# PeterFWS/Structure-PLP-SLAM

Measured on AMD Instinct MI355X. Metric: frames/sec ORB+LSD extract+match, 640x480 TUM-RGBD, 1/2/4/8 GPU, higher is better.
Workload: dtype u8

## Files before the change

structure-plp-slam_amd/csrc/match_kernels.hip:

```cpp
#include <hip/hip_runtime.h>
#include <stdint.h>
#include <cstdlib>

#include "libstdcxx_sort.hpp"
#include "plp_barrier.hpp"
#include "match_device.hpp"
#include "plp_common.hpp"
#include "xcd_map.hpp"

namespace plp {

__device__ __forceinline__ int floor_d(double v) { int i = (int)v; return i - (i > v); }
__device__ __forceinline__ int ceil_d(double v) { int i = (int)v; return i + (i < v); }

__device__ __forceinline__ unsigned hamming256(const uint4& a0, const uint4& a1, const uint4& b0, const uint4& b1) {
    return __popc(a0.x ^ b0.x) + __popc(a0.y ^ b0.y) + __popc(a0.z ^ b0.z) + __popc(a0.w ^ b0.w) +
           __popc(a1.x ^ b1.x) + __popc(a1.y ^ b1.y) + __popc(a1.z ^ b1.z) + __popc(a1.w ^ b1.w);
}

__device__ __forceinline__ unsigned long long wave_min_u64(unsigned long long v) {
#pragma unroll
    for (int o = 32; o > 0; o >>= 1) {
        const unsigned lo = __shfl_xor((unsigned)v, o), hi = __shfl_xor((unsigned)(v >> 32), o);
        const unsigned long long w = ((unsigned long long)hi << 32) | lo;
        v = w < v ? w : v;
    }
    return v;
}

struct QueryCtx {
    float rx, ry, mg, xr, xr2;
    int min_level, max_level, min_cx, max_cx, min_cy, max_cy;
    double l0, l1, l2, lden;
    double rdx, rdy;
    int group;
    unsigned pred;
    double g0, g1, g2, gden;
    double b1x, b1y, b1z, thr;
    bool stereo;
    bool windowed, empty, line;
};
__device__ __forceinline__ bool is_line_mode(int mode) { return mode == PLP_MATCH_MODE_LANDMARKS_LINE || mode == PLP_MATCH_MODE_LAST_FRAME_LINE || mode == PLP_MATCH_MODE_FUSE_LINE; }
__device__ __forceinline__ bool is_group_mode(int mode) { return mode == PLP_MATCH_MODE_BOW || mode == PLP_MATCH_MODE_TRIANGULATION; }
__device__ __forceinline__ bool is_last_frame_mode(int mode) { return mode == PLP_MATCH_MODE_LAST_FRAME || mode == PLP_MATCH_MODE_LAST_FRAME_LINE; }

template <int FAM>
__device__ __forceinline__ int fam_mode(int m) {
    if constexpr (FAM == kFamLine) return m == PLP_MATCH_MODE_LANDMARKS_LINE ? PLP_MATCH_MODE_LANDMARKS_LINE : PLP_MATCH_MODE_LAST_FRAME_LINE;
    else if constexpr (FAM == kFamGroup) return m == PLP_MATCH_MODE_BOW ? PLP_MATCH_MODE_BOW : PLP_MATCH_MODE_TRIANGULATION;
    else if constexpr (FAM == kFamPoint) return m == PLP_MATCH_MODE_LANDMARKS ? PLP_MATCH_MODE_LANDMARKS : m == PLP_MATCH_MODE_LAST_FRAME ? PLP_MATCH_MODE_LAST_FRAME : PLP_MATCH_MODE_BRUTE_FORCE;
    else if constexpr (FAM == kFamGrid) return m == PLP_MATCH_MODE_LANDMARKS ? PLP_MATCH_MODE_LANDMARKS : PLP_MATCH_MODE_LAST_FRAME;
    else return m;
}

__device__ __forceinline__ int query_direction(const MatchProblem& P, int b) {
    typedef const __attribute__((address_space(1))) int32_t* g_i32;
    return P.directions ? ((g_i32)P.directions)[b] : P.direction;
}

template <int FAM = kFamAny>
__device__ __forceinline__ QueryCtx make_query(const MatchProblem& P, int q, int b, int dir) {
    const int mode = fam_mode<FAM>(P.mode);
    const size_t qoff = (size_t)b * P.m_cap;
    const float* reproj = P.q_reproj ? P.q_reproj + qoff * 2 : nullptr;
    const float* q_xr = P.q_x_right ? P.q_x_right + qoff : nullptr;
    const int32_t* q_level = P.q_level ? P.q_level + qoff : nullptr;
    QueryCtx c{};
    c.windowed = mode != PLP_MATCH_MODE_BRUTE_FORCE && !is_group_mode(mode);
    c.line = is_line_mode(mode);
    if (is_group_mode(mode)) c.group = P.q_group[qoff + q];
    if (mode == PLP_MATCH_MODE_TRIANGULATION) {
        const double* bq = P.q_bearing + (qoff + q) * 3;
        c.b1x = bq[0]; c.b1y = bq[1]; c.b1z = bq[2];
        c.stereo = q_xr && 0 <= q_xr[q];
        c.thr = (0.2 * 3.14159265358979323846 / 180.0) * (double)P.scale_factors[q_level[q] & 15];
    }
    if (!c.windowed) return c;
    const int lvl = q_level[q];
    const int lvl_tab = min(max(lvl, 0), max(P.num_levels, 1) - 1);
    if (c.line) {
        c.mg = __fmul_rn(P.margin, P.scale_factors[lvl_tab]);
        double x1, y1, x2, y2;
        if (mode == PLP_MATCH_MODE_FUSE_LINE) {
            const double* a = P.q_reproj_d + (qoff + q) * 2; const double* e = P.q_reproj2_d + (qoff + q) * 2;
            x1 = (float)a[0]; y1 = (float)a[1]; x2 = (float)e[0]; y2 = (float)e[1];
            c.g0 = a[1] * 1.0 - 1.0 * e[1]; c.g1 = 1.0 * e[0] - a[0] * 1.0; c.g2 = a[0] * e[1] - a[1] * e[0];
            c.gden = sqrt(c.g0 * c.g0 + c.g1 * c.g1);
        } else {
            const float* r2 = P.q_reproj2 + qoff * 2;
            x1 = reproj[2 * q]; y1 = reproj[2 * q + 1]; x2 = r2[2 * q]; y2 = r2[2 * q + 1];
        }
        c.l0 = y1 * 1.0 - 1.0 * y2; c.l1 = 1.0 * x2 - x1 * 1.0; c.l2 = x1 * y2 - y1 * x2;
        c.lden = sqrt(c.l0 * c.l0 + c.l1 * c.l1);
        c.xr = q_xr ? q_xr[q] : -1.f;
        c.xr2 = P.q_x_right2 ? P.q_x_right2[qoff + q] : -1.f;
        if (mode == PLP_MATCH_MODE_FUSE_LINE) { c.min_level = -1; c.max_level = -1; }
        else if (mode == PLP_MATCH_MODE_LANDMARKS_LINE || P.level_window == 1) { c.min_level = lvl - 1; c.max_level = lvl; }
        else if (P.level_window == 2) { c.min_level = lvl - 1; c.max_level = lvl + 1; }
        else {
            if (dir == 1) { c.min_level = lvl; c.max_level = P.num_levels_lsd; }
            else if (dir == 2) { c.min_level = 0; c.max_level = lvl + 1; }
            else { c.min_level = lvl - 1; c.max_level = lvl + 1; }
        }
        c.empty = false;
        return c;
    }
    if (mode == PLP_MATCH_MODE_FUSE) {
        const double* rd = P.q_reproj_d + qoff * 2;
        c.rdx = rd[2 * q]; c.rdy = rd[2 * q + 1];
        c.rx = (float)c.rdx; c.ry = (float)c.rdy;
        c.pred = (unsigned)lvl;
    } else { c.rx = reproj[2 * q]; c.ry = reproj[2 * q + 1]; }
    c.mg = __fmul_rn(P.margin, P.scale_factors[lvl_tab]);
    c.xr = q_xr ? q_xr[q] : -1.f;
    if (mode == PLP_MATCH_MODE_LANDMARKS || (mode == PLP_MATCH_MODE_LAST_FRAME && P.level_window == 1)) { c.min_level = lvl - 1; c.max_level = lvl; }
    else if (mode == PLP_MATCH_MODE_FUSE) { c.min_level = -1; c.max_level = -1; }
    else if (P.level_window == 2) { c.min_level = lvl - 1; c.max_level = lvl + 1; }
    else {
        if (dir == 1) { c.min_level = lvl; c.max_level = P.num_levels - 1; }
        else if (dir == 2) { c.min_level = 0; c.max_level = lvl; }
        else { c.min_level = lvl - 1; c.max_level = lvl + 1; }
    }
    c.min_cx = max(0, floor_d((double)__fsub_rn(__fsub_rn(c.rx, P.grid_min_x), c.mg) * P.inv_cell_w));
    c.max_cx = min(P.grid_cols - 1, ceil_d((double)__fadd_rn(__fsub_rn(c.rx, P.grid_min_x), c.mg) * P.inv_cell_w));
    c.min_cy = max(0, floor_d((double)__fsub_rn(__fsub_rn(c.ry, P.grid_min_y), c.mg) * P.inv_cell_h));
    c.max_cy = min(P.grid_rows - 1, ceil_d((double)__fadd_rn(__fsub_rn(c.ry, P.grid_min_y), c.mg) * P.inv_cell_h));
    c.empty = P.grid_cols <= c.min_cx || c.max_cx < 0 || P.grid_rows <= c.min_cy || c.max_cy < 0;
    if (mode == PLP_MATCH_MODE_LAST_FRAME && (P.flags & PLP_MATCH_FLAG_UNSIGNED_LEVEL) && lvl == 0) c.empty = true;
    return c;
}

struct LineTarget { float sx, sy, ex, ey; int octave; bool occ; float xr, xr2; unsigned kp_oct; };
template <int FAM = kFamAny>
__device__ __forceinline__ bool line_gate(const MatchProblem& P, const QueryCtx& c, const LineTarget& T, bool has_xr) {
    const int mode = fam_mode<FAM>(P.mode);
    const float dsp = (float)(((double)T.sx * c.l0 + (double)T.sy * c.l1 + c.l2) / c.lden);
    const float dep = (float)(((double)T.ex * c.l0 + (double)T.ey * c.l1 + c.l2) / c.lden);
    if (fabsf(dsp) > c.mg || fabsf(dep) > c.mg) return false;
    const bool check_level = (0 < c.min_level) || (0 <= c.max_level);
    if (check_level) {
        if (T.octave < c.min_level) return false;
        if (c.max_level > 0 && T.octave > c.max_level) return false;
    }
    if (T.occ) return false;
    if (mode == PLP_MATCH_MODE_LAST_FRAME_LINE && P.is_rgbd && has_xr && P.t_x_right2) {
        const float a = T.xr, b2 = T.xr2;
        if (a > 0 && b2 > 0 && (c.mg < fabsf(__fsub_rn(c.xr, a)) || c.mg < fabsf(__fsub_rn(c.xr2, b2)))) return false;
    }
    return true;
}

template <int FAM = kFamAny>
__device__ __forceinline__ unsigned long long candidate_key(const MatchProblem& P, const QueryCtx& c, int t, const plp_keypoint* kps,
                                                           const uint8_t* t_desc, const float* t_xr, const uint8_t* t_occ,
                                                           const uint4& q0, const uint4& q1) {
    const int mode = fam_mode<FAM>(P.mode);
    unsigned order = (unsigned)t, oct = 0;
    if (is_group_mode(mode)) {
        const size_t tb = (size_t)(t_desc - P.t_desc) / 32;
// ... 403 lines not shown
#pragma unroll
                for (int e = kMatchK - 1; e > 0; --e) { const uint32_t lo = min(ovf[e], ovf[e - 1]), hi = max(ovf[e], ovf[e - 1]); ovf[e - 1] = lo; ovf[e] = hi; }
            }
        };
        int passed = 0;
        float rx = 0.f, ry = 0.f, mg = 0.f, qxr = 0.f;
        uint32_t win = 1u, lvls = 255u << 16;
        int i = 0, i1 = 0;
        uint4 q0 = make_uint4(0u, 0u, 0u, 0u), q1 = q0;
        if (active) {
            const QueryCtx c = make_query(P, q, b, s_dir);
            if (!c.empty) {
                const uint4* qd = reinterpret_cast<const uint4*>(P.q_desc + ((size_t)b * P.q_desc_stride + q) * 32);
                q0 = qd[0]; q1 = qd[1];
                rx = c.rx; ry = c.ry; mg = c.mg; qxr = c.xr;
                win = (uint32_t)c.min_cx | ((uint32_t)c.max_cx << 8) | ((uint32_t)c.min_cy << 16) | ((uint32_t)c.max_cy << 24);
                lvls = (uint32_t)min(max(c.min_level, 0), 256) | ((c.max_level < 0 ? 255u : (uint32_t)min(c.max_level, 255)) << 16);
            }
        }
        bool wave_more;
        do {
            uint32_t pend[kLanePend / 2];
#pragma unroll
            for (int k = 0; k < kLanePend / 2; ++k) pend[k] = 0u;
            int nc = 0;
            for (;;) {
                if (i >= i1) {
                    const int col = (int)(win & 0xffu);
                    if (col <= (int)((win >> 8) & 0xffu)) {
                        i = cs[col * rows + (int)((win >> 16) & 0xffu)]; i1 = cs[col * rows + (int)(win >> 24) + 1];
                        ++win;
                    }
                } else {
                    const int p = i++;
                    const float2 sp = t_xy(p);
                    const uint32_t oct = t_to(p) >> 16;
                    bool ok = (lvls & 0xffffu) <= oct && oct <= (lvls >> 16) && fabsf(__fsub_rn(sp.x, rx)) < mg && fabsf(__fsub_rn(sp.y, ry)) < mg;
                    if (ok && has_xr) {
                        const float xr = t_xr(p);
                        ok = !(0 < xr && mg < fabsf(__fsub_rn(qxr, xr)));
                    }
                    if (ok) {
                        const uint32_t v = (uint32_t)p << (16 * (nc & 1));
#pragma unroll
                        for (int k = 0; k < kLanePend / 2; ++k) pend[k] |= (nc >> 1) == k ? v : 0u;
                        ++nc;
                    }
                }
                wave_more = __builtin_amdgcn_ballot_w64(i < i1 || (win & 0xffu) <= ((win >> 8) & 0xffu)) != 0ull;
                if (!wave_more || __builtin_amdgcn_ballot_w64(nc == kLanePend) != 0ull) break;
            }
            auto slot_pos = [&](int j) -> int { return (int)((pend[j >> 1] >> (16 * (j & 1))) & 0xffffu); };
            auto gather = [&](int j, uint4& a0, uint4& a1) {
                if (j < nc) {
                    const uint4* d = reinterpret_cast<const uint4*>(t_desc + 32 * (size_t)(t_to(slot_pos(j)) & 0xffffu));
                    a0 = d[0]; a1 = d[1];
                }
            };
            uint4 a0 = make_uint4(0u, 0u, 0u, 0u), a1 = a0;
            gather(0, a0, a1);
#pragma unroll
            for (int j = 0; j < kLanePend; ++j) {
                if (__builtin_amdgcn_ballot_w64(j < nc) == 0ull) break;
                uint4 b0 = a0, b1 = a1;
                if (j + 1 < kLanePend) gather(j + 1, b0, b1);
                if (j < nc) insert((hamming256(q0, q1, a0, a1) << 16) | (uint32_t)slot_pos(j));
                a0 = b0; a1 = b1;
            }
            passed += nc;
        } while (wave_more);
        if (!in_range) continue;
        uint32_t e[kMatchK];
#pragma unroll
        for (int k = 0; k < kMatchK; ++k) {
            e[k] = 0xffffffffu;
            if (top[k] != 0xffffffffu) {
                const uint32_t to = t_to((int)(top[k] & 0xffffu));
                e[k] = ((top[k] >> 16) << 20) | (((to >> 16) & 15u) << 16) | (to & 0xffffu);
            }
        }
        static_assert(kMatchK == 8, "two 16-byte stores per query");
        uint4* out = reinterpret_cast<uint4*>(P.klist + ((size_t)b * P.m_cap + q) * kMatchK);
        out[0] = make_uint4(e[0], e[1], e[2], e[3]);
        out[1] = make_uint4(e[4], e[5], e[6], e[7]);
        P.kcount[(size_t)b * P.m_cap + q] = active ? passed : -1;
        if (passed > kMatchK) {
#pragma unroll
            for (int k = 0; k < kMatchK; ++k) {
                e[k] = 0xffffffffu;
                if (ovf[k] != 0xffffffffu) {
                    const uint32_t to = t_to((int)(ovf[k] & 0xffffu));
                    e[k] = ((ovf[k] >> 16) << 20) | (((to >> 16) & 15u) << 16) | (to & 0xffffu);
                }
            }
            uint4* out2 = reinterpret_cast<uint4*>(P.klist2 + ((size_t)b * P.m_cap + q) * kMatchK);
            out2[0] = make_uint4(e[0], e[1], e[2], e[3]);
            out2[1] = make_uint4(e[4], e[5], e[6], e[7]);
        }
    }
}

__global__ __launch_bounds__(256) void k_match_topk_lds(MatchProblem P) {
    extern __shared__ __attribute__((aligned(16))) uint8_t smem[];
    const int tid = threadIdx.x, lane = tid & 63, wv = __builtin_amdgcn_readfirstlane(tid >> 6), b = blockIdx.y;
    const int m = P.q_counts ? min(P.q_counts[b], P.m_cap) : P.m_cap;
    const int q_begin = blockIdx.x * kQueriesPerBlock;
    if (q_begin >= m) return;
    const int n = P.t_counts ? min(P.t_counts[b], P.n_cap) : P.n_cap;
    const uint8_t* t_desc = P.t_desc + (size_t)b * P.n_cap * 32;
    uint4* sdesc = reinterpret_cast<uint4*>(smem);
    {
        const uint4* src = reinterpret_cast<const uint4*>(t_desc);
        for (int i = tid; i < 2 * n; i += 256) sdesc[i] = src[i];
    }
    wg_barrier();
    const uint8_t* q_valid = P.q_valid ? P.q_valid + (size_t)b * P.m_cap : nullptr;
    for (int q = q_begin + wv; q < min(m, q_begin + kQueriesPerBlock); q += 4) {
        uint32_t* klist = P.klist + ((size_t)b * P.m_cap + q) * kMatchK;
        int32_t* kcount = P.kcount + (size_t)b * P.m_cap + q;
        if (q_valid && !q_valid[q]) { if (lane == 0) *kcount = -1; continue; }
        const uint4* qd = reinterpret_cast<const uint4*>(P.q_desc + ((size_t)b * P.q_desc_stride + q) * 32);
        const uint4 q0 = qd[0], q1 = qd[1];
        unsigned long long top[kMatchK];
#pragma unroll
        for (int i = 0; i < kMatchK; ++i) top[i] = ~0ull;
        int passed = 0;
        for (int t = lane; t < n; t += 64) {
            const unsigned dist = hamming256(q0, q1, sdesc[2 * t], sdesc[2 * t + 1]);
            ++passed;
            topk_insert(top, ((unsigned long long)dist << 32) | ((unsigned long long)(unsigned)t << 4));
        }
#pragma unroll
        for (int o = 32; o > 0; o >>= 1) passed += __shfl_xor(passed, o);
        topk_merge_store(top, lane, klist);
        if (lane == 0) *kcount = passed;
    }
}

template <int FAM = kFamAny>
__device__ __forceinline__ bool accept(const MatchProblem& P, unsigned best, int best_lvl, unsigned second, int second_lvl) {
    const int mode = fam_mode<FAM>(P.mode);
    if (mode == PLP_MATCH_MODE_LANDMARKS || mode == PLP_MATCH_MODE_LANDMARKS_LINE) {
        if (!(best <= 100u)) return false;
        if (best_lvl == second_lvl && (float)best > __fmul_rn(P.lowe_ratio, (float)second)) return false;
        return true;
    }
    if (is_last_frame_mode(mode)) return best <= (P.hamm_dist_thr > 0 ? (unsigned)P.hamm_dist_thr : 100u);
    if (mode == PLP_MATCH_MODE_TRIANGULATION) return true;
    if (50u < best) return false;
    if (__fmul_rn(P.lowe_ratio, (float)second) < (float)best) return false;
    return true;
}

template <bool kSorted, int FAM = kFamAny>
__device__ __forceinline__ void match_resolve_body(const MatchProblem& P) {
    const int mode = fam_mode<FAM>(P.mode);
    extern __shared__ int32_t lds[];
    __shared__ int s_changed, s_num, s_hist[32], s_valid_bin[32], s_full_n, s_claim_tmp[256], s_sort_ws[48];
    __shared__ unsigned s_sort_idx[32];
    __shared__ int s_dir;
    const int tid = threadIdx.x, lane = tid & 63, wv = __builtin_amdgcn_readfirstlane(tid >> 6), b = blockIdx.x;
    const int m = P.q_counts ? min(P.q_counts[b], P.m_cap) : P.m_cap;
    const int n = P.t_counts ? min(P.t_counts[b], P.n_cap) : P.n_cap;
    int32_t* owner_final = lds;
    int32_t* owner_prev = lds + P.n_cap;
    int32_t* owner_next = lds + 2 * P.n_cap;
    const uint32_t* klist = P.klist + (size_t)b * P.m_cap * kMatchK;
    const int32_t* kcount = P.kcount + (size_t)b * P.m_cap;
    int32_t* claim = P.claim + (size_t)b * P.m_cap;
    const uint8_t* has_obs = P.q_has_obs ? P.q_has_obs + (size_t)b * P.m_cap : nullptr;
    const plp_keypoint* kps = P.t_kps ? P.t_kps + (size_t)b * P.n_cap : nullptr;
    const uint8_t* t_desc = P.t_desc + (size_t)b * P.n_cap * 32;
    const float* t_xr = P.t_x_right ? P.t_x_right + (size_t)b * P.n_cap : nullptr;
    const uint8_t* t_occ = P.t_occupied ? P.t_occupied + (size_t)b * P.n_cap : nullptr;
    int32_t* out = P.out_match + (size_t)b * P.n_cap;

    for (int t = tid; t < n; t += 256) { owner_final[t] = 0x7fffffff; out[t] = -1; }
    for (int q = tid; q < m; q += 256) claim[q] = -1;
    if (is_last_frame_mode(mode) && tid == 0) s_dir = query_direction(P, b);
    wg_barrier();

    int32_t* full_list = P.full_list + (size_t)b * P.m_cap;
    const int need = (is_last_frame_mode(mode) || mode == PLP_MATCH_MODE_TRIANGULATION) ? 1 : 2;
    const bool blocks_always = !has_obs || mode == PLP_MATCH_MODE_BRUTE_FORCE || is_group_mode(mode);
    const unsigned t_flip = mode == PLP_MATCH_MODE_TRIANGULATION ? 0xffffu : 0u;
    constexpr bool use_sorted = kSorted;
    const StagedTarget* sorted = P.sorted + (size_t)b * P.n_cap;
    const float* sorted_xr = P.sorted_xr + (size_t)b * P.n_cap;
    const uint16_t* g_cell_start = P.cell_start + (size_t)b * kCellStride;
    auto taken = [&](int t, int q, int) -> bool { return owner_final[t] != 0x7fffffff || owner_prev[t] < q; };
    {
        for (int chunk_start = 0; chunk_start < m; chunk_start += 256) {
          const int q = chunk_start + tid;
          int my_claim = -1;
          for (int t = tid; t < n; t += 256) owner_prev[t] = 0x7fffffff;
          constexpr int kList = kSorted ? 2 * kMatchK : kMatchK;
          uint32_t e8[kList];
          int cnt = 0;
          if (q < m) {
              cnt = kcount[q];
              const uint4* kp = reinterpret_cast<const uint4*>(klist + (size_t)q * kMatchK);
              const uint4 lo = kp[0], hi = kp[1];
              e8[0] = lo.x; e8[1] = lo.y; e8[2] = lo.z; e8[3] = lo.w; e8[4] = hi.x; e8[5] = hi.y; e8[6] = hi.z; e8[7] = hi.w;
              if constexpr (kSorted) {
#pragma unroll
                  for (int k = kMatchK; k < kList; ++k) e8[k] = 0xffffffffu;
                  if (cnt > kMatchK) {
                      const uint4* kp2 = reinterpret_cast<const uint4*>(P.klist2 + ((size_t)b * P.m_cap + q) * kMatchK);
                      const uint4 lo2 = kp2[0], hi2 = kp2[1];
                      e8[8] = lo2.x; e8[9] = lo2.y; e8[10] = lo2.z; e8[11] = lo2.w; e8[12] = hi2.x; e8[13] = hi2.y; e8[14] = hi2.z; e8[15] = hi2.w;
                  }
              }
          }
          for (int inner = 0; inner <= 256; ++inner) {
            if (tid == 0) { s_full_n = 0; s_changed = 0; }
            for (int t = tid; t < n; t += 256) owner_next[t] = 0x7fffffff;
            wg_barrier();
            int new_claim = -1;
            bool decided = false;
            if (q < m) {
                if (cnt <= 0) decided = true;
                else {
                    const int have = min(cnt, kList);
                    unsigned best = 256, second = 256;
                    int best_lvl = -1, second_lvl = -1, best_t = -1, found = 0;
#pragma unroll
                    for (int e = 0; e < kList; ++e) {
                        if (e >= have || found >= need) continue;
                        const int t = (int)((e8[e] & 0xffff) ^ t_flip);
                        if (taken(t, q, chunk_start)) continue;
                        if (found == 0) { best = e8[e] >> 20; best_lvl = (int)((e8[e] >> 16) & 15); best_t = t; }
                        else { second = e8[e] >> 20; second_lvl = (int)((e8[e] >> 16) & 15); }
                        ++found;
                    }
                    bool rescan = found < need && cnt > kList;
                    if (rescan && mode != PLP_MATCH_MODE_TRIANGULATION) {
                        const unsigned d8 = e8[kList - 1] >> 20;
                        const bool lm = mode == PLP_MATCH_MODE_LANDMARKS || mode == PLP_MATCH_MODE_LANDMARKS_LINE;
                        const unsigned thr = (lm || is_last_frame_mode(mode)) ? (is_last_frame_mode(mode) && P.hamm_dist_thr > 0 ? (unsigned)P.hamm_dist_thr : 100u) : 50u;
                        if (found == 0) { if (d8 > thr) rescan = false; }
                        else if (best > thr) rescan = false;
                        else if (lm) { if (!((float)best > __fmul_rn(P.lowe_ratio, (float)d8))) { rescan = false; second = d8; second_lvl = -2; } }
                        else if (!(__fmul_rn(P.lowe_ratio, (float)d8) < (float)best)) { rescan = false; second = d8; }
                    }
                    if (rescan) full_list[atomicAdd(&s_full_n, 1)] = q;
                    else { decided = true; if (found > 0 && accept<FAM>(P, best, best_lvl, second, second_lvl)) new_claim = best_t; }
                }
            }
            wg_barrier();
            const int nf = s_full_n;
            if (tid == 0 && P.dbg && nf) atomicAdd(&P.dbg[0], nf);
            for (int f = wv; f < nf; f += 4) {
                const int fq = full_list[f];
                const QueryCtx c = make_query<FAM>(P, fq, b, s_dir);
                const uint4* qd = reinterpret_cast<const uint4*>(P.q_desc + ((size_t)b * P.q_desc_stride + fq) * 32);
                const uint4 q0 = qd[0], q1 = qd[1];
                unsigned long long k0 = ~0ull, k1 = ~0ull;
                if constexpr (use_sorted) {
                    if (!c.empty) {
                        const bool check_level = (0 < c.min_level) || (0 <= c.max_level);
                        for (int col = c.min_cx; col <= c.max_cx; ++col) {
                            const int i0 = g_cell_start[col * P.grid_rows + c.min_cy], i1 = g_cell_start[col * P.grid_rows + c.max_cy + 1];
                            for (int i = i0 + lane; i < i1; i += 64) {
                                const StagedTarget s = sorted[i];
                                const int oct = (int)(s.packed & 0xff);
                                if (check_level) {
                                    if (oct < c.min_level) continue;
                                    if (0 <= c.max_level && c.max_level < oct) continue;
                                }
                                if (!(fabsf(__fsub_rn(s.x, c.rx)) < c.mg && fabsf(__fsub_rn(s.y, c.ry)) < c.mg)) continue;
                                if (t_xr) {
                                    const float xr = sorted_xr[i];
                                    if (0 < xr && c.mg < fabsf(__fsub_rn(c.xr, xr))) continue;
                                }
                                if (taken((int)s.t, fq, chunk_start)) continue;
                                const uint4* d = reinterpret_cast<const uint4*>(t_desc + 32 * (size_t)s.t);
                                const unsigned dist = hamming256(q0, q1, d[0], d[1]);
                                const unsigned long long key = ((unsigned long long)dist << 32) | ((unsigned long long)(unsigned)i << 4) | (unsigned)(oct & 15);
                                if (key < k0) { k1 = k0; k0 = key; } else if (key < k1) k1 = key;
                            }
                        }
                    }
                } else if (!(c.windowed && c.empty)) {
                    for (int t = lane; t < n; t += 64) {
                        if (taken(t, fq, chunk_start)) continue;
                        const unsigned long long key = candidate_key<FAM>(P, c, t, kps, t_desc, t_xr, t_occ, q0, q1);
                        if (key < k0) { k1 = k0; k0 = key; } else if (key < k1) k1 = key;
                    }
                }
                const unsigned long long g0 = wave_min_u64(k0);
                const unsigned long long g1 = wave_min_u64(k0 == g0 ? k1 : k0);
                if (lane == 0) {
                    int nc = -1;
                    if (g0 != ~0ull) {
                        const unsigned second = g1 != ~0ull ? (unsigned)(g1 >> 32) : 256u;
                        const int second_lvl = g1 != ~0ull ? (int)(g1 & 15) : -1;
                        if (accept<FAM>(P, (unsigned)(g0 >> 32), (int)(g0 & 15), second, second_lvl))
                            nc = use_sorted ? (int)sorted[(g0 >> 4) & 0xffff].t : (int)(((g0 >> 4) & 0xffff) ^ t_flip);
                    }
                    s_claim_tmp[fq - chunk_start] = nc;
                }
            }
            wg_barrier();
            if (q < m) {
                if (!decided) new_claim = s_claim_tmp[tid];
                if (my_claim != new_claim) { my_claim = new_claim; s_changed = 1; }
                if (new_claim >= 0 && (blocks_always || has_obs[q])) atomicMin(&owner_next[new_claim], q);
            }
            wg_barrier();
            { int32_t* t = owner_prev; owner_prev = owner_next; owner_next = t; }
            const int changed = s_changed;
            wg_barrier();
            if (!changed) break;
          }
          if (tid == 0 && P.dbg) atomicAdd(&P.dbg[1], 1);
          if (q < m) {
              claim[q] = my_claim;
              if (my_claim >= 0 && (blocks_always || has_obs[q])) atomicMin(&owner_final[my_claim], q);
          }
          wg_barrier();
        }
    }

    if (tid == 0) s_num = 0;
    for (int i = tid; i < 32; i += 256) { s_hist[i] = 0; s_valid_bin[i] = 0; }
    wg_barrier();
    const bool angle_check = P.check_orientation && (mode == PLP_MATCH_MODE_LAST_FRAME || mode == PLP_MATCH_MODE_BRUTE_FORCE || is_group_mode(mode));
    const float* q_angle = P.q_angle ? P.q_angle + (size_t)b * P.m_cap : nullptr;
    const float* t_angle = P.t_angle ? P.t_angle + (size_t)b * P.n_cap : nullptr;
    auto bin_of = [&](int q, int t) -> int {
        const float ta = kps ? kps[t].angle : t_angle[t];
        float delta = (mode == PLP_MATCH_MODE_LAST_FRAME || is_group_mode(mode)) ? __fsub_rn(q_angle[q], ta) : __fsub_rn(ta, q_angle[q]);
        if (delta < 0.0) delta = (float)((double)delta + 360.0);
        if (360.0 <= delta) delta = (float)((double)delta - 360.0);
        const int bin = __float2int_rn(__fmul_rn(delta, 1.0f / 30));
        return (unsigned)bin > 31u ? 31 : bin;
    };
    int my = 0;
    for (int q = tid; q < m; q += 256) {
        const int t = claim[q];
        if (t < 0) continue;
        ++my;
        atomicMax(&out[t], q);
        if (angle_check) atomicAdd(&s_hist[min(bin_of(q, t), 31)], 1);
    }
    if (my) atomicAdd(&s_num, my);
    wg_barrier();
    if (angle_check) {
        if (tid == 0) {
            libstdcxx::index_sort_by_size(s_hist, 30, s_sort_idx, s_sort_ws);
            for (int r = 0; r < 3; ++r) s_valid_bin[s_sort_idx[r]] = 1;
        }
        wg_barrier();
        int bad = 0;
        for (int q = tid; q < m; q += 256) {
            const int t = claim[q];
            if (t < 0) continue;
            if (!s_valid_bin[min(bin_of(q, t), 31)]) { out[t] = (P.flags & PLP_MATCH_FLAG_MARK_INVALIDATED) ? -2 : -1; ++bad; }
        }
        if (bad) atomicSub(&s_num, bad);
        wg_barrier();
    }
    if (tid == 0) P.out_num[b] = s_num;
}
__global__ __launch_bounds__(256) __attribute__((amdgpu_waves_per_eu(4, 8))) void k_match_resolve_sorted(MatchProblem P) { match_resolve_body<true, kFamGrid>(P); }
template <int FAM>
__global__ __launch_bounds__(256) void k_match_resolve_generic(MatchProblem P) { match_resolve_body<false, FAM>(P); }

__global__ __launch_bounds__(256) void k_hamming_matrix(const uint8_t* __restrict__ qd, int nq, const uint8_t* __restrict__ td, int nt,
                                                        uint16_t* __restrict__ dist) {
    __shared__ uint32_t sq[64 * 9], st[64 * 9];
    const int tid = threadIdx.x;
    const int q0 = blockIdx.y * 64, t0 = blockIdx.x * 64;
    for (int i = tid; i < 64 * 8; i += 256) {
        const int r = i >> 3, w = i & 7;
        sq[r * 9 + w] = q0 + r < nq ? reinterpret_cast<const uint32_t*>(qd)[(size_t)(q0 + r) * 8 + w] : 0u;
        st[r * 9 + w] = t0 + r < nt ? reinterpret_cast<const uint32_t*>(td)[(size_t)(t0 + r) * 8 + w] : 0u;
    }
    wg_barrier();
    const int tx = tid & 63, ty = __builtin_amdgcn_readfirstlane(tid >> 6);
    uint32_t tv[8];
#pragma unroll
    for (int w = 0; w < 8; ++w) tv[w] = st[tx * 9 + w];
    for (int r = ty; r < 64; r += 4) {
        unsigned d = 0;
#pragma unroll
        for (int w = 0; w < 8; ++w) d += __popc(sq[r * 9 + w] ^ tv[w]);
        if (q0 + r < nq && t0 + tx < nt) dist[(size_t)(q0 + r) * nt + t0 + tx] = (uint16_t)d;
    }
}

__global__ __launch_bounds__(256) void k_match_fuse(MatchProblem P) {
    const int lane = threadIdx.x & 63, b = blockIdx.y;
    const int q = blockIdx.x * 4 + __builtin_amdgcn_readfirstlane((int)(threadIdx.x >> 6));
    const int m = P.q_counts ? min(P.q_counts[b], P.m_cap) : P.m_cap;
    if (q >= m) return;
    int32_t* out = P.out_query_best + (size_t)b * P.m_cap + q;
    const uint8_t* q_valid = P.q_valid ? P.q_valid + (size_t)b * P.m_cap : nullptr;
    if (q_valid && !q_valid[q]) { if (lane == 0) *out = -1; return; }
    const int n = P.t_counts ? min(P.t_counts[b], P.n_cap) : P.n_cap;
    const plp_keypoint* kps = P.t_kps + (size_t)b * P.n_cap;
    const uint8_t* t_desc = P.t_desc + (size_t)b * P.n_cap * 32;
    const float* t_xr = P.t_x_right ? P.t_x_right + (size_t)b * P.n_cap : nullptr;
    const QueryCtx c = make_query(P, q, b, query_direction(P, b));
    const uint4* qd = reinterpret_cast<const uint4*>(P.q_desc + ((size_t)b * P.q_desc_stride + q) * 32);
    const uint4 q0 = qd[0], q1 = qd[1];
    unsigned long long best = ~0ull;
    if (!c.empty)
        for (int t = lane; t < n; t += 64) {
            const unsigned long long key = candidate_key(P, c, t, kps, t_desc, t_xr, nullptr, q0, q1);
            best = key < best ? key : best;
        }
    best = wave_min_u64(best);
    const unsigned thr = P.hamm_dist_thr > 0 ? (unsigned)P.hamm_dist_thr : 50u;
    if (lane == 0) *out = (best != ~0ull && (unsigned)(best >> 32) <= thr) ? (int32_t)((best >> 4) & 0xffff) : -1;
}

__global__ __launch_bounds__(64) void k_match_area(AreaArgs A) {
    __shared__ int hist[32], valid_bin[32], sort_ws[48];
    __shared__ unsigned sort_idx[32];
    const int lane = threadIdx.x;
    uint32_t* mdist = A.scratch;
    int32_t* m1in2 = reinterpret_cast<int32_t*>(A.scratch + A.n2);
    for (int i = lane; i < A.n2; i += 64) { mdist[i] = 256u; m1in2[i] = -1; }
    for (int i = lane; i < A.n1; i += 64) A.matched_2_in_1[i] = -1;
    if (lane < 32) { hist[lane] = 0; valid_bin[lane] = 0; }
    __builtin_amdgcn_fence(__ATOMIC_ACQ_REL, "workgroup");
    __builtin_amdgcn_wave_barrier();
    auto bin_of = [&](int i1, int i2) -> int {
        float delta = __fsub_rn(A.kps1[i1].angle, A.kps2[i2].angle);
        if (delta < 0.0) delta = (float)((double)delta + 360.0);
        if (360.0 <= delta) delta = (float)((double)delta - 360.0);
        const int bin = __float2int_rn(__fmul_rn(delta, 1.0f / 30));
        return (unsigned)bin > 31u ? 31 : bin;
    };
    for (int i1 = 0; i1 < A.n1; ++i1) {
        const plp_keypoint k1 = A.kps1[i1];
        if (0 < k1.octave) continue;
        const float rx = A.prev_pts[2 * i1], ry = A.prev_pts[2 * i1 + 1], mg = A.margin;
        const int min_cx = max(0, floor_d((double)__fsub_rn(__fsub_rn(rx, A.grid_min_x), mg) * A.inv_cell_w));
        const int max_cx = min(A.grid_cols - 1, ceil_d((double)__fadd_rn(__fsub_rn(rx, A.grid_min_x), mg) * A.inv_cell_w));
        const int min_cy = max(0, floor_d((double)__fsub_rn(__fsub_rn(ry, A.grid_min_y), mg) * A.inv_cell_h));
        const int max_cy = min(A.grid_rows - 1, ceil_d((double)__fadd_rn(__fsub_rn(ry, A.grid_min_y), mg) * A.inv_cell_h));
        if (A.grid_cols <= min_cx || max_cx < 0 || A.grid_rows <= min_cy || max_cy < 0) continue;
        const uint4* qd = reinterpret_cast<const uint4*>(A.desc1 + 32 * (size_t)i1);
        const uint4 q0 = qd[0], q1 = qd[1];
        unsigned long long k0 = ~0ull, k1k = ~0ull;
        for (int t = lane; t < A.n2; t += 64) {
            const plp_keypoint k = A.kps2[t];
            const int cx = floor_d((double)__fsub_rn(k.x, A.grid_min_x) * A.inv_cell_w), cy = floor_d((double)__fsub_rn(k.y, A.grid_min_y) * A.inv_cell_h);
            if (cx < 0 || cx >= A.grid_cols || cy < 0 || cy >= A.grid_rows) continue;
            if (cx < min_cx || cx > max_cx || cy < min_cy || cy > max_cy) continue;
            if (k.octave < 0 || 0 < k.octave) continue;
            if (!(fabsf(__fsub_rn(k.x, rx)) < mg && fabsf(__fsub_rn(k.y, ry)) < mg)) continue;
            const uint4* d = reinterpret_cast<const uint4*>(A.desc2 + 32 * (size_t)t);
            const unsigned dist = hamming256(q0, q1, d[0], d[1]);
            if (mdist[t] <= dist) continue;
            const unsigned long long key = ((unsigned long long)dist << 32) | ((unsigned long long)(((unsigned)(cx * A.grid_rows + cy) << 16) | (unsigned)t));
            if (key < k0) { k1k = k0; k0 = key; } else if (key < k1k) k1k = key;
        }
        const unsigned long long g0 = wave_min_u64(k0);
        const unsigned long long g1 = wave_min_u64(k0 == g0 ? k1k : k0);
        if (g0 == ~0ull) continue;
        const unsigned best = (unsigned)(g0 >> 32), second = g1 != ~0ull ? (unsigned)(g1 >> 32) : 256u;
        if (50u < best) continue;
        if (__fmul_rn((float)second, A.lowe_ratio) < (float)best) continue;
        const int best_i2 = (int)(g0 & 0xffff);
        if (lane == 0) {
            const int prev_i1 = m1in2[best_i2];
            if (0 <= prev_i1) A.matched_2_in_1[prev_i1] = -1;
            A.matched_2_in_1[i1] = best_i2;
            m1in2[best_i2] = i1;
            mdist[best_i2] = best;
            if (A.check_orientation) hist[bin_of(i1, best_i2)] += 1;
        }
        __builtin_amdgcn_fence(__ATOMIC_ACQ_REL, "workgroup");
        __builtin_amdgcn_wave_barrier();
    }
    if (A.check_orientation && lane == 0) {
        libstdcxx::index_sort_by_size(hist, 30, sort_idx, sort_ws);
        for (int r = 0; r < 3; ++r) valid_bin[sort_idx[r]] = 1;
    }
    __builtin_amdgcn_fence(__ATOMIC_ACQ_REL, "workgroup");
    __builtin_amdgcn_wave_barrier();
    int cnt = 0;
    for (int i1 = lane; i1 < A.n1; i1 += 64) {
        const int i2 = A.matched_2_in_1[i1];
        if (i2 < 0) continue;
        if (A.check_orientation && !valid_bin[bin_of(i1, i2)]) { A.matched_2_in_1[i1] = -1; continue; }
        ++cnt;
        A.prev_pts[2 * i1] = A.kps2[i2].x; A.prev_pts[2 * i1 + 1] = A.kps2[i2].y;
    }
#pragma unroll
    for (int o = 32; o > 0; o >>= 1) cnt += __shfl_xor(cnt, o);
    if (lane == 0) *A.num_matches = cnt;
}

void launch_match_area(hipStream_t st, const AreaArgs& A) { hipLaunchKernelGGL(k_match_area, dim3(1), dim3(64), 0, st, A); }

static bool is_line_mode_host(int mode) { return mode == PLP_MATCH_MODE_LANDMARKS_LINE || mode == PLP_MATCH_MODE_LAST_FRAME_LINE || mode == PLP_MATCH_MODE_FUSE_LINE; }

MatchPlan plan_match(const MatchProblem& P, int B) {
    MatchPlan pl{kTopkNone, kFamAny, 0, kResolveNone, 0};
    if (P.mode == PLP_MATCH_MODE_FUSE || P.mode == PLP_MATCH_MODE_FUSE_LINE) { pl.topk = kTopkFuse; return pl; }
    const bool windowed = P.mode == PLP_MATCH_MODE_LANDMARKS || P.mode == PLP_MATCH_MODE_LAST_FRAME;
    const bool line = is_line_mode_host(P.mode) || P.mode == PLP_MATCH_MODE_BOW || P.mode == PLP_MATCH_MODE_TRIANGULATION;
    pl.family = is_line_mode_host(P.mode) ? kFamLine : (P.mode == PLP_MATCH_MODE_BOW || P.mode == PLP_MATCH_MODE_TRIANGULATION) ? kFamGroup : kFamPoint;
    pl.staged = windowed ? (size_t)P.lds_targets * (P.t_x_right ? 16 : 12) + 2 * kCellStride : (size_t)P.n_cap * 32;
    pl.resolve = kResolveGeneric;
    if (!line && windowed && pl.staged <= 64 * 1024 && P.grid_cols <= 255 && P.grid_rows <= 255) {
        pl.topk = kTopkCells;
        pl.family = kFamGrid;
        pl.resolve = kResolveSorted;
        pl.qpb = B >= 64 ? 512 : 32;
    } else if (!line && !windowed && pl.staged <= 64 * 1024) {
        pl.topk = kTopkLds;
// ... 95 lines not shown
```

Baseline: 100,000.

## Restructure match resolve loop: fewer barriers, bitmask picks, dead-chunk skip, fused tally

```diff
diff --git a/structure-plp-slam_amd/csrc/match_kernels.hip b/structure-plp-slam_amd/csrc/match_kernels.hip
--- a/structure-plp-slam_amd/csrc/match_kernels.hip
+++ b/structure-plp-slam_amd/csrc/match_kernels.hip
@@ -5,6 +5,7 @@
 #include "libstdcxx_sort.hpp"
 #include "plp_barrier.hpp"
 #include "match_device.hpp"
+#include "match_resolve.hpp"
 #include "plp_common.hpp"
 #include "xcd_map.hpp"
 
@@ -714,14 +715,55 @@
     return true;
 }
 
+#ifdef PLP_RESOLVE_PROF
+__device__ unsigned long long g_rs_prof[16][16];
+#define RS_PROF_LAP(k) do { const long long rs_now = clock64(); rs_acc[k] += (unsigned long long)(rs_now - rs_t); rs_t = rs_now; } while (0)
+#define RS_PROF_ADD(v, n) ((v) += (n))
+#define RS_PROF_SET(v, n) ((v) = (n))
+#define RS_PROF_DEPTH(d)                                                                        \
+    do {                                                                                        \
+        int rs_d = (d);                                                                         \
+        for (int o = 32; o > 0; o >>= 1) rs_d = max(rs_d, __shfl_xor(rs_d, o));                 \
+        rs_depth_max = max(rs_depth_max, rs_d); rs_depth_sum += rs_d;                           \
+    } while (0)
+#define RS_PROF_REPORT()                                                                        \
+    do {                                                                                        \
+        if (tid == 0) {                                                                         \
+            unsigned long long* R = g_rs_prof[P.mode & 15];                                     \
+            for (int k = 0; k < 9; ++k) atomicAdd(&R[k], rs_acc[k]);                            \
+            atomicAdd(&R[9], 1ull); atomicAdd(&R[10], (unsigned long long)rs_chunks); atomicAdd(&R[11], (unsigned long long)rs_iters); \
+            atomicMax(&R[12], (unsigned long long)rs_depth_max); atomicAdd(&R[13], (unsigned long long)rs_depth_sum);                  \
+            atomicAdd(&R[14], (unsigned long long)rs_dead);                                     \
+        }                                                                                       \
+    } while (0)
+extern "C" int plp_debug_resolve_phases(unsigned long long* out, int reset) {
+    if (out && hipMemcpyFromSymbol(out, HIP_SYMBOL(g_rs_prof), sizeof(g_rs_prof)) != hipSuccess) return 1;
+    if (reset) { static const unsigned long long zero[16][16] = {}; if (hipMemcpyToSymbol(HIP_SYMBOL(g_rs_prof), zero, sizeof(zero)) != hipSuccess) return 1; }
+    return 0;
+}
+#else
+#define RS_PROF_LAP(k) ((void)0)
+#define RS_PROF_ADD(v, n) ((void)0)
+#define RS_PROF_SET(v, n) ((void)0)
+#define RS_PROF_DEPTH(d) ((void)0)
+#define RS_PROF_REPORT() ((void)0)
+#endif
+
 template <bool kSorted, int FAM = kFamAny>
 __device__ __forceinline__ void match_resolve_body(const MatchProblem& P) {
     const int mode = fam_mode<FAM>(P.mode);
     extern __shared__ int32_t lds[];
-    __shared__ int s_changed, s_num, s_hist[32], s_valid_bin[32], s_full_n, s_claim_tmp[256], s_sort_ws[48];
+    __shared__ int s_changed[2], s_num, s_hist[32], s_valid_bin[32], s_full_n[2], s_claim_tmp[256], s_sort_ws[48];
     __shared__ unsigned s_sort_idx[32];
+    constexpr int kLiveChunks = 1024;
+    __shared__ unsigned s_live[kLiveChunks / 32];
     __shared__ int s_dir;
     const int tid = threadIdx.x, lane = tid & 63, wv = __builtin_amdgcn_readfirstlane(tid >> 6), b = blockIdx.x;
+#ifdef PLP_RESOLVE_PROF
+    long long rs_t = clock64();
+    unsigned long long rs_acc[9] = {};
+    int rs_chunks = 0, rs_iters = 0, rs_depth_max = 0, rs_depth_sum = 0, rs_dead = 0, rs_walk = 0;
+#endif
     const int m = P.q_counts ? min(P.q_counts[b], P.m_cap) : P.m_cap;
     const int n = P.t_counts ? min(P.t_counts[b], P.n_cap) : P.n_cap;
     int32_t* owner_final = lds;
@@ -737,10 +779,18 @@
     const uint8_t* t_occ = P.t_occupied ? P.t_occupied + (size_t)b * P.n_cap : nullptr;
     int32_t* out = P.out_match + (size_t)b * P.n_cap;
 
-    for (int t = tid; t < n; t += 256) { owner_final[t] = 0x7fffffff; out[t] = -1; }
-    for (int q = tid; q < m; q += 256) claim[q] = -1;
+    for (int t = tid; t < n; t += 256) { owner_final[t] = 0x7fffffff; owner_prev[t] = 0x7fffffff; owner_next[t] = 0x7fffffff; out[t] = -1; }
+    for (int i = tid; i < kLiveChunks / 32; i += 256) s_live[i] = 0u;
+    if (tid == 0) { s_full_n[0] = 0; s_full_n[1] = 0; s_changed[0] = 0; s_changed[1] = 0; s_num = 0; }
+    for (int i = tid; i < 32; i += 256) { s_hist[i] = 0; s_valid_bin[i] = 0; }
     if (is_last_frame_mode(mode) && tid == 0) s_dir = query_direction(P, b);
     wg_barrier();
+    for (int c0 = 0, k = 0; c0 < m && k < kLiveChunks; c0 += 256, ++k) {
+        const bool live = c0 + tid < m && kcount[c0 + tid] > 0;
+        if (__builtin_amdgcn_ballot_w64(live) != 0ull && lane == 0) atomicOr(&s_live[k >> 5], 1u << (k & 31));
+    }
+    wg_barrier();
+    RS_PROF_LAP(0);
 
     int32_t* full_list = P.full_list + (size_t)b * P.m_cap;
     const int need = (is_last_frame_mode(mode) || mode == PLP_MATCH_MODE_TRIANGULATION) ? 1 : 2;
@@ -751,11 +801,37 @@
     const float* sorted_xr = P.sorted_xr + (size_t)b * P.n_cap;
     const uint16_t* g_cell_start = P.cell_start + (size_t)b * kCellStride;
     auto taken = [&](int t, int q, int) -> bool { return owner_final[t] != 0x7fffffff || owner_prev[t] < q; };
+    const bool angle_check = P.check_orientation && (mode == PLP_MATCH_MODE_LAST_FRAME || mode == PLP_MATCH_MODE_BRUTE_FORCE || is_group_mode(mode));
+    const float* q_angle = P.q_angle ? P.q_angle + (size_t)b * P.m_cap : nullptr;
+    const float* t_angle = P.t_angle ? P.t_angle + (size_t)b * P.n_cap : nullptr;
+    auto bin_of = [&](int q, int t) -> int {
+        const float ta = kps ? kps[t].angle : t_angle[t];
+        float delta = (mode == PLP_MATCH_MODE_LAST_FRAME || is_group_mode(mode)) ? __fsub_rn(q_angle[q], ta) : __fsub_rn(ta, q_angle[q]);
+        if (delta < 0.0) delta = (float)((double)delta + 360.0);
+        if (360.0 <= delta) delta = (float)((double)delta - 360.0);
+        const int bin = __float2int_rn(__fmul_rn(delta, 1.0f / 30));
+        return (unsigned)bin > 31u ? 31 : bin;
+    };
+    int my = 0;
+    unsigned long long kept0 = ~0ull, kept1 = ~0ull;
+    int dbg_rescans = 0, dbg_rounds = 0;
+    const bool lm_mode = mode == PLP_MATCH_MODE_LANDMARKS || mode == PLP_MATCH_MODE_LANDMARKS_LINE;
+    const plp_resolve::Rules rules{need, t_flip, mode != PLP_MATCH_MODE_TRIANGULATION, lm_mode,
+                                   (lm_mode || is_last_frame_mode(mode)) ? (is_last_frame_mode(mode) && P.hamm_dist_thr > 0 ? (unsigned)P.hamm_dist_thr : 100u) : 50u, P.lowe_ratio};
     {
-        for (int chunk_start = 0; chunk_start < m; chunk_start += 256) {
+        int chunk_no = 0;
+        for (int chunk_start = 0; chunk_start < m; chunk_start += 256, ++chunk_no) {
           const int q = chunk_start + tid;
+          const int chunk_live = chunk_no >= kLiveChunks ? 1 : __builtin_amdgcn_readfirstlane((int)((s_live[chunk_no >> 5] >> (chunk_no & 31)) & 1u));
+          if (!chunk_live) {
+              if (q < m) claim[q] = -1;
+              dbg_rounds += tid == 0;
+              RS_PROF_ADD(rs_chunks, 1);
+              RS_PROF_ADD(rs_dead, 1);
+              RS_PROF_LAP(5);
+              continue;
+          }
           int my_claim = -1;
-          for (int t = tid; t < n; t += 256) owner_prev[t] = 0x7fffffff;
           constexpr int kList = kSorted ? 2 * kMatchK : kMatchK;
           uint32_t e8[kList];
           int cnt = 0;
@@ -774,44 +850,38 @@
                   }
               }
           }
+          const int have = q < m ? max(0, min(cnt, kList)) : 0;
+#pragma unroll
+          for (int e = 0; e < kList; ++e) e8[e] = e < have ? e8[e] : t_flip;
+          const bool blocks = q < m && (blocks_always || has_obs[q]);
+          unsigned fmask = 0u;
+#pragma unroll
+          for (int e = 0; e < kList; ++e) fmask |= (unsigned)(owner_final[(int)((e8[e] & 0xffff) ^ t_flip)] == 0x7fffffff) << e;
+          RS_PROF_LAP(1);
           for (int inner = 0; inner <= 256; ++inner) {
-            if (tid == 0) { s_full_n = 0; s_changed = 0; }
-            for (int t = tid; t < n; t += 256) owner_next[t] = 0x7fffffff;
+            const int par = inner & 1;
+            RS_PROF_ADD(rs_iters, 1);
+            RS_PROF_SET(rs_walk, 0);
+            unsigned open = fmask;
+            if (inner > 0) {
+                unsigned held = 0u;
+#pragma unroll
+                for (int e = 0; e < kList; ++e) held |= (unsigned)(owner_prev[(int)((e8[e] & 0xffff) ^ t_flip)] < q) << e;
+                open &= ~held;
+            }
+            int new_claim = -1;
+            bool decided = true;
+            if (q < m && cnt > 0) {
+                const plp_resolve::Pick pk = plp_resolve::pick_mask<kList>(e8, cnt, rules, open);
+                RS_PROF_SET(rs_walk, pk.last);
+                if (pk.rescan) { decided = false; full_list[atomicAdd(&s_full_n[par], 1)] = q; }
+                else if (pk.found > 0 && accept<FAM>(P, pk.best, pk.best_lvl, pk.second, pk.second_lvl)) new_claim = pk.best_t;
+            }
+            RS_PROF_DEPTH(rs_walk);
             wg_barrier();
-            int new_claim = -1;
-            bool decided = false;
-            if (q < m) {
-                if (cnt <= 0) decided = true;
-                else {
-                    const int have = min(cnt, kList);
-                    unsigned best = 256, second = 256;
-                    int best_lvl = -1, second_lvl = -1, best_t = -1, found = 0;
-#pragma unroll
-                    for (int e = 0; e < kList; ++e) {
-                        if (e >= have || found >= need) continue;
-                        const int t = (int)((e8[e] & 0xffff) ^ t_flip);
-                        if (taken(t, q, chunk_start)) continue;
-                        if (found == 0) { best = e8[e] >> 20; best_lvl = (int)((e8[e] >> 16) & 15); best_t = t; }
-                        else { second = e8[e] >> 20; second_lvl = (int)((e8[e] >> 16) & 15); }
-                        ++found;
-                    }
-                    bool rescan = found < need && cnt > kList;
-                    if (rescan && mode != PLP_MATCH_MODE_TRIANGULATION) {
-                        const unsigned d8 = e8[kList - 1] >> 20;
-                        const bool lm = mode == PLP_MATCH_MODE_LANDMARKS || mode == PLP_MATCH_MODE_LANDMARKS_LINE;
-                        const unsigned thr = (lm || is_last_frame_mode(mode)) ? (is_last_frame_mode(mode) && P.hamm_dist_thr > 0 ? (unsigned)P.hamm_dist_thr : 100u) : 50u;
-                        if (found == 0) { if (d8 > thr) rescan = false; }
-                        else if (best > thr) rescan = false;
-                        else if (lm) { if (!((float)best > __fmul_rn(P.lowe_ratio, (float)d8))) { rescan = false; second = d8; second_lvl = -2; } }
-                        else if (!(__fmul_rn(P.lowe_ratio, (float)d8) < (float)best)) { rescan = false; second = d8; }
-                    }
-                    if (rescan) full_list[atomicAdd(&s_full_n, 1)] = q;
-                    else { decided = true; if (found > 0 && accept<FAM>(P, best, best_lvl, second, second_lvl)) new_claim = best_t; }
-                }
-            }
-            wg_barrier();
-            const int nf = s_full_n;
-            if (tid == 0 && P.dbg && nf) atomicAdd(&P.dbg[0], nf);
+            RS_PROF_LAP(2);
+            const int nf = __builtin_amdgcn_readfirstlane(s_full_n[par]);
+            dbg_rescans += tid == 0 ? nf : 0;
             for (int f = wv; f < nf; f += 4) {
                 const int fq = full_list[f];
                 const QueryCtx c = make_query<FAM>(P, fq, b, s_dir);
@@ -863,67 +933,77 @@
                     s_claim_tmp[fq - chunk_start] = nc;
                 }
             }
-            wg_barrier();
+            if (nf) wg_barrier();
+            RS_PROF_LAP(3);
             if (q < m) {
                 if (!decided) new_claim = s_claim_tmp[tid];
-                if (my_claim != new_claim) { my_claim = new_claim; s_changed = 1; }
-                if (new_claim >= 0 && (blocks_always || has_obs[q])) atomicMin(&owner_next[new_claim], q);
-            }
+                if (my_claim != new_claim) { my_claim = new_claim; s_changed[par] = 1; }
+                if (new_claim >= 0 && blocks) atomicMin(&owner_next[new_claim], q);
+            }
+            if (tid == 0) { s_full_n[par ^ 1] = 0; s_changed[par ^ 1] = 0; }
             wg_barrier();
             { int32_t* t = owner_prev; owner_prev = owner_next; owner_next = t; }
-            const int changed = s_changed;
-            wg_barrier();
-            if (!changed) break;
+            const int changed = __builtin_amdgcn_readfirstlane(s_changed[par]);
+            if (!changed) { RS_PROF_LAP(4); break; }
+            for (int t = tid; t < n; t += 256) owner_next[t] = 0x7fffffff;
+            RS_PROF_LAP(4);
           }
-          if (tid == 0 && P.dbg) atomicAdd(&P.dbg[1], 1);
+          RS_PROF_ADD(rs_chunks, 1);
+          dbg_rounds += tid == 0;
           if (q < m) {
               claim[q] = my_claim;
-              if (my_claim >= 0 && (blocks_always || has_obs[q])) atomicMin(&owner_final[my_claim], q);
+              if (my_claim >= 0) {
+                  if (blocks) atomicMin(&owner_final[my_claim], q);
+                  ++my;
+                  atomicMax(&out[my_claim], q);
+                  if (angle_check) {
+                      const int bin = min(bin_of(q, my_claim), 31);
+                      atomicAdd(&s_hist[bin], 1);
+                      const unsigned long long put = (unsigned long long)(0xff ^ bin) << (8 * (chunk_no & 7));
+                      if (chunk_no < 8) kept0 ^= put; else if (chunk_no < 16) kept1 ^= put;
+                  }
+              }
           }
+          for (int t = tid; t < n; t += 256) { owner_prev[t] = 0x7fffffff; owner_next[t] = 0x7fffffff; }
+          if (tid == 0) { s_full_n[0] = 0; s_full_n[1] = 0; }
           wg_barrier();
-        }
-    }
-
-    if (tid == 0) s_num = 0;
-    for (int i = tid; i < 32; i += 256) { s_hist[i] = 0; s_valid_bin[i] = 0; }
-    wg_barrier();
-    const bool angle_check = P.check_orientation && (mode == PLP_MATCH_MODE_LAST_FRAME || mode == PLP_MATCH_MODE_BRUTE_FORCE || is_group_mode(mode));
-    const float* q_angle = P.q_angle ? P.q_angle + (size_t)b * P.m_cap : nullptr;
-    const float* t_angle = P.t_angle ? P.t_angle + (size_t)b * P.n_cap : nullptr;
-    auto bin_of = [&](int q, int t) -> int {
-        const float ta = kps ? kps[t].angle : t_angle[t];
-        float delta = (mode == PLP_MATCH_MODE_LAST_FRAME || is_group_mode(mode)) ? __fsub_rn(q_angle[q], ta) : __fsub_rn(ta, q_angle[q]);
-        if (delta < 0.0) delta = (float)((double)delta + 360.0);
-        if (360.0 <= delta) delta = (float)((double)delta - 360.0);
-        const int bin = __float2int_rn(__fmul_rn(delta, 1.0f / 30));
-        return (unsigned)bin > 31u ? 31 : bin;
-    };
-    int my = 0;
-    for (int q = tid; q < m; q += 256) {
-        const int t = claim[q];
-        if (t < 0) continue;
-        ++my;
-        atomicMax(&out[t], q);
-        if (angle_check) atomicAdd(&s_hist[min(bin_of(q, t), 31)], 1);
-    }
+          RS_PROF_LAP(5);
+        }
+    }
+
     if (my) atomicAdd(&s_num, my);
     wg_barrier();
+    RS_PROF_LAP(6);
     if (angle_check) {
         if (tid == 0) {
             libstdcxx::index_sort_by_size(s_hist, 30, s_sort_idx, s_sort_ws);
             for (int r = 0; r < 3; ++r) s_valid_bin[s_sort_idx[r]] = 1;
         }
         wg_barrier();
-        int bad = 0;
-        for (int q = tid; q < m; q += 256) {
-            const int t = claim[q];
-            if (t < 0) continue;
-            if (!s_valid_bin[min(bin_of(q, t), 31)]) { out[t] = (P.flags & PLP_MATCH_FLAG_MARK_INVALIDATED) ? -2 : -1; ++bad; }
+        RS_PROF_LAP(7);
+        int bad = 0, k = 0;
+        for (int q = tid; q < m; q += 256, ++k) {
+            int bin;
+            if (k < 16) {
+                bin = (int)(((k < 8 ? kept0 : kept1) >> (8 * (k & 7))) & 0xffull);
+                if (bin == 0xff) continue;
+            } else {
+                const int t = claim[q];
+                if (t < 0) continue;
+                bin = min(bin_of(q, t), 31);
+            }
+            if (!s_valid_bin[bin]) { out[claim[q]] = (P.flags & PLP_MATCH_FLAG_MARK_INVALIDATED) ? -2 : -1; ++bad; }
         }
         if (bad) atomicSub(&s_num, bad);
         wg_barrier();
     }
     if (tid == 0) P.out_num[b] = s_num;
+    if (tid == 0 && P.dbg) {
+        if (dbg_rescans) atomicAdd(&P.dbg[0], dbg_rescans);
+        if (dbg_rounds) atomicAdd(&P.dbg[1], dbg_rounds);
+    }
+    RS_PROF_LAP(8);
+    RS_PROF_REPORT();
 }
 __global__ __launch_bounds__(256) __attribute__((amdgpu_waves_per_eu(4, 8))) void k_match_resolve_sorted(MatchProblem P) { match_resolve_body<true, kFamGrid>(P); }
 template <int FAM>
diff --git a/structure-plp-slam_amd/csrc/match_resolve.hpp b/structure-plp-slam_amd/csrc/match_resolve.hpp
--- /dev/null
+++ b/structure-plp-slam_amd/csrc/match_resolve.hpp
@@ -0,0 +1,83 @@
+#pragma once
+#include <stdint.h>
+
+#if defined(__HIPCC__) || defined(__CUDACC__)
+#define PLP_RESOLVE_HD __host__ __device__ __forceinline__
+#else
+#define PLP_RESOLVE_HD inline
+#endif
+
+namespace plp_resolve {
+
+PLP_RESOLVE_HD float mul_rn(float a, float b) {
+#if defined(__HIP_DEVICE_COMPILE__)
+    return __fmul_rn(a, b);
+#else
+    volatile float r = a * b;
+    return r;
+#endif
+}
+
+struct Rules {
+    int need;
+    unsigned t_flip;
+    bool d8_rules;
+    bool lm;
+    unsigned thr;
+    float lowe_ratio;
+};
+
+struct Pick {
+    unsigned best, second;
+    int best_lvl, second_lvl, best_t, found;
+    bool rescan;
+    int last;
+};
+
+PLP_RESOLVE_HD void dry_list(Pick& p, unsigned d8, const Rules& R) {
+    if (!R.d8_rules) return;
+    if (p.found == 0) { if (d8 > R.thr) p.rescan = false; }
+    else if (p.best > R.thr) p.rescan = false;
+    else if (R.lm) { if (!((float)p.best > mul_rn(R.lowe_ratio, (float)d8))) { p.rescan = false; p.second = d8; p.second_lvl = -2; } }
+    else if (!(mul_rn(R.lowe_ratio, (float)d8) < (float)p.best)) { p.rescan = false; p.second = d8; }
+}
+
+template <int kList, class Taken>
+PLP_RESOLVE_HD Pick pick_walk(const uint32_t (&e8)[kList], int cnt, const Rules& R, Taken taken) {
+    Pick p{256u, 256u, -1, -1, -1, 0, false, 0};
+    const int have = cnt < kList ? cnt : kList;
+    for (int e = 0; e < kList; ++e) {
+        if (e >= have || p.found >= R.need) continue;
+        p.last = e + 1;
+        const int t = (int)((e8[e] & 0xffff) ^ R.t_flip);
+        if (taken(t)) continue;
+        if (p.found == 0) { p.best = e8[e] >> 20; p.best_lvl = (int)((e8[e] >> 16) & 15); p.best_t = t; }
+        else { p.second = e8[e] >> 20; p.second_lvl = (int)((e8[e] >> 16) & 15); }
+        ++p.found;
+    }
+    p.rescan = p.found < R.need && cnt > kList;
+    if (p.rescan) dry_list(p, e8[kList - 1] >> 20, R);
+    return p;
+}
+
+template <int kList>
+PLP_RESOLVE_HD Pick pick_mask(const uint32_t (&e8)[kList], int cnt, const Rules& R, unsigned free_mask) {
+    static_assert(kList <= 16, "one bit per entry");
+    Pick p{256u, 256u, -1, -1, -1, 0, false, 0};
+    const int have = cnt < kList ? (cnt < 0 ? 0 : cnt) : kList;
+    const unsigned m0 = free_mask & ((1u << have) - 1u);
+    const unsigned m1 = m0 & (m0 - 1u);
+    const int i0 = m0 ? __builtin_ctz(m0) : -1;
+    const int i1 = (R.need > 1 && m1) ? __builtin_ctz(m1) : -1;
+    uint32_t v0 = 0u, v1 = 0u;
+#pragma unroll
+    for (int e = 0; e < kList; ++e) { v0 = e == i0 ? e8[e] : v0; v1 = e == i1 ? e8[e] : v1; }
+    if (i0 >= 0) { p.best = v0 >> 20; p.best_lvl = (int)((v0 >> 16) & 15); p.best_t = (int)((v0 & 0xffff) ^ R.t_flip); p.found = 1; }
+    if (i1 >= 0) { p.second = v1 >> 20; p.second_lvl = (int)((v1 >> 16) & 15); p.found = 2; }
+    p.last = p.found >= R.need ? (R.need > 1 ? i1 : i0) + 1 : have;
+    p.rescan = p.found < R.need && cnt > kList;
+    if (p.rescan) dry_list(p, e8[kList - 1] >> 20, R);
+    return p;
+}
+
+}
```

Result: no change. 100,000 (-0.0%).
